# sandyz1000/face-landmark-detector

Measured on AMD Instinct MI355X. Metric: faces/sec (whole node), 256x256 batch inference: fused preprocess + FCN-8 forward + softmax + top-4 landmark decode + similarity/alignment warp, higher is better.
Workload: dtype f32; 1 GPU; BASELINE configs[1]: batch=64/GPU 256x256x3 uint8 crops, fcn_8(68) vanilla encoder fp32, random-init weights (seed 2), decode top-4 thresh 0, align to 256x256; global_batch=64, parallelism=dp1

## Files before the change

### face-landmark-detector_amd/csrc/flm_api.hip

```cpp
#include <cmath>
#include <cstdarg>
#include <cstdio>
#include <cstring>

#include "flm_common.h"

namespace flm {

static thread_local char g_err[512] = "";

void set_error(const char* fmt, ...) {
  va_list ap;
  va_start(ap, fmt);
  vsnprintf(g_err, sizeof(g_err), fmt, ap);
  va_end(ap);
}

int hip_fail(hipError_t e, const char* what) {
  set_error("HIP error %d (%s) at %s", (int)e, hipGetErrorString(e), what);
  return FLM_ERR_HIP;
}

struct Knob {
  const char* key;
// ... 6 lines not shown
    {"bf16_lds_dma", {1}, nullptr, nullptr},
    {"bf16_mfma16", {1}, nullptr, nullptr},
    {"bf16_halo_mfma16", {1}, nullptr, nullptr},
    {"f32_two_level", {1}, nullptr, nullptr},
    {"f32_lean_tile", {1}, nullptr, nullptr},
    {"bf16_group_n", {0}, [](int v) { return v >= 0 && v <= 32 && !(v & (v - 1)); }, "0 or a power of two <= 32"},
    {"bf16_conv3_halo", {1}, nullptr, nullptr},
    {"bf16_score1x1", {1}, nullptr, nullptr},
    {"bf16_fused_tail", {1}, nullptr, nullptr},
    {"decode_lds_dma", {1}, nullptr, nullptr},
    {"posmajor_order", {1}, nullptr, nullptr},
    {"warp_rows", {1}, [](int v) { return v == 0 || v == 1 || v == 4; }, "0, 1 or 4"},
    {"up3_cand8", {1}, [](int v) { return v >= 0 && v <= 7; }, "in [0,7]"},
    {"up3_cand8_rows", {0}, [](int v) { return v >= 0 && v <= 8 && !(v & (v - 1)); }, "0, 1, 2, 4 or 8"},
    {"up3_wreg", {0}, [](int v) { return v == 0 || v == 1; }, "0 or 1"},
};
static_assert(sizeof(g_knobs) / sizeof(g_knobs[0]) == KNOB_COUNT, "one row per KnobId");
int tuning(KnobId id) { return g_knobs[id].value.load(std::memory_order_relaxed); }
static Knob* find_knob(const char* who, const char* key) {
  for (Knob& k : g_knobs)
    if (!strcmp(k.key, key)) return &k;
  set_error("%s: unknown key '%s'", who, key);
  return nullptr;
}

struct ProfRec {
  const char* name;
  hipEvent_t a, b;
};
static ProfRec* g_prof = nullptr;
// ... 182 lines not shown
    t.ho = 2 * hi; t.wo = 2 * wi; t.ldy = L.g.Cp;
  }
  return t;
}

}

using namespace flm;

extern "C" {

int flm_abi_version(void) { return FLM_ABI_VERSION; }

int flm_debug_query(const char* key, int arg) {
  if (key && !strcmp(key, "igemm_occupancy")) return igemm_occupancy((size_t)arg);
  return -1;
}

int flm_set_tuning(const char* key, int value) {
  if (!key) return FLM_ERR_ARG;
  if (!strcmp(key, "none")) return FLM_OK;
  if (!strcmp(key, "landmark_candidates") || !strcmp(key, "candidate_sub_phases") || !strcmp(key, "candidate_cap_div")) {
    set_error("flm_set_tuning: '%s' changes the workspace layout and is a per-call option now: pass flm_forward_opts to "
              "flm_fcn_workspace_bytes_opts / flm_fcn_forward_opts", key);
    return FLM_ERR_ARG;
  }
  Knob* k = find_knob("flm_set_tuning", key);
  if (!k) return FLM_ERR_ARG;
  if (k->valid && !k->valid(value)) {
    set_error("flm_set_tuning: %s must be %s", key, k->domain);
// ... 1475 lines not shown
```

### face-landmark-detector_amd/csrc/flm_common.h

```cpp
#pragma once

#include <hip/hip_runtime.h>
#include <stddef.h>
#include <stdint.h>

#include <atomic>
#include <mutex>

#include "flm.h"

namespace flm {

void set_error(const char* fmt, ...);
int hip_fail(hipError_t e, const char* what);

#define FLM_HIP(call)                                            \
  do {                                                           \
    hipError_t e_ = (call);                                      \
    if (e_ != hipSuccess) return ::flm::hip_fail(e_, #call);     \
  } while (0)

#define FLM_LAUNCH_CHECK(what)                                   \
  do {                                                           \
    hipError_t e_ = hipGetLastError();                           \
// ... 93 lines not shown
  size_t splitk_bytes;
  size_t probs;
  size_t decode;
  size_t sub, tau, cand, cand_cnt;
  int cand_cap;
  int cand_sub;
  size_t total;
  int oh, ow;
};
Fcn8Ws fcn8_ws_layout(int n, int h, int w, int C, int dtype, int out_mode, int decode_mode, int n_points,
                      int arch = 0, const flm_forward_opts* opts = nullptr);

enum KnobId {
  KNOB_BF16_BIG_TILES, KNOB_BF16_LDS_DMA, KNOB_BF16_MFMA16, KNOB_BF16_HALO_MFMA16, KNOB_F32_TWO_LEVEL, KNOB_F32_LEAN_TILE,
  KNOB_BF16_GROUP_N, KNOB_BF16_CONV3_HALO, KNOB_BF16_SCORE1X1, KNOB_BF16_FUSED_TAIL, KNOB_DECODE_LDS_DMA,
  KNOB_POSMAJOR_ORDER, KNOB_WARP_ROWS, KNOB_UP3_CAND8, KNOB_UP3_CAND8_ROWS, KNOB_UP3_WREG, KNOB_COUNT
};
int tuning(KnobId id);

int launch_pack_fcn(hipStream_t s, const flm_fcn_params& p, int C, const Fcn8Pack& L, char* blob);

int launch_enc1(hipStream_t s, const void* x, int in_format, int n, int h, int w, const float* w1p,
                const float* scale, const float* shift, void* f1, int out_bf16, int pool);

struct IgemmDesc {
  const void* x;
  const void* wt;
  const float* scale;
  const float* shift;
  void* y;
  int bf16;
  int out_f32;
  int n, h, w, cin;
  int cout;
  int coutpad;
  int ldc;
  int kh, kw, pad;
  int relu, pool, posmajor;
  int stride;
  const void* res;
  float* splitk_ws;
  size_t splitk_ws_bytes;
};
int launch_igemm(hipStream_t s, const IgemmDesc& d);
int igemm_occupancy(size_t lds_bytes);
int launch_seg_fused_bf16(hipStream_t s, const float* fuse4, const void* w4_packed, const void* f3, const void* w3,
                          const float* scale3, const float* shift3, float* seg, int n, int h4, int w4d, int C, int Cp,
                          int G, int cin3, int coutpad3);

struct ConvTDesc {
  const float* x;
  const void* wf;
  const float* skip;
  void* y;
  int n, hi, wi;
  int ho, wo;
  int s;
  int ldy;
  int epilogue;
  ConvTGeom g;
// ... 163 lines not shown
```

### face-landmark-detector_amd/csrc/flm_igemm.hip

```cpp
#include <type_traits>
#include <vector>

#include "flm_igemm_args.h"

#ifndef FLM_IGEMM_VAR
#define FLM_IGEMM_VAR 0
#endif

namespace flm {

typedef float f32x16 __attribute__((ext_vector_type(16)));
typedef __bf16 bf16x8 __attribute__((ext_vector_type(8)));

constexpr int BM = 128, BN = 128, BK = 32;
constexpr int TILE_F = BM * BK;

__device__ __forceinline__ int swz(int row, int chunk) { return row * BK + ((chunk ^ ((row >> 1) & 7)) << 2); }

__device__ __forceinline__ float f4c(const float4& v, int i) { return i == 0 ? v.x : (i == 1 ? v.y : (i == 2 ? v.z : v.w)); }

template <bool BF, int IDX>
__device__ __forceinline__ void mfma_slot(const float4& a0, const float4& a1, const float4& b0, const float4& b1,
                                          f32x16& c00, f32x16& c01, f32x16& c10, f32x16& c11) {
  if constexpr (BF) {
    const float4& av = (IDX >> 1) ? a1 : a0;
    const float4& bv = (IDX & 1) ? b1 : b0;
    const bf16x8 af = __builtin_bit_cast(bf16x8, av), bfr = __builtin_bit_cast(bf16x8, bv);
    if constexpr (IDX == 0) c00 = __builtin_amdgcn_mfma_f32_32x32x16_bf16(af, bfr, c00, 0, 0, 0);
    if constexpr (IDX == 1) c01 = __builtin_amdgcn_mfma_f32_32x32x16_bf16(af, bfr, c01, 0, 0, 0);
    if constexpr (IDX == 2) c10 = __builtin_amdgcn_mfma_f32_32x32x16_bf16(af, bfr, c10, 0, 0, 0);
    if constexpr (IDX == 3) c11 = __builtin_amdgcn_mfma_f32_32x32x16_bf16(af, bfr, c11, 0, 0, 0);
  } else {
    c00 = __builtin_amdgcn_mfma_f32_32x32x2f32(f4c(a0, IDX), f4c(b0, IDX), c00, 0, 0, 0);
    c01 = __builtin_amdgcn_mfma_f32_32x32x2f32(f4c(a0, IDX), f4c(b1, IDX), c01, 0, 0, 0);
    c10 = __builtin_amdgcn_mfma_f32_32x32x2f32(f4c(a1, IDX), f4c(b0, IDX), c10, 0, 0, 0);
    c11 = __builtin_amdgcn_mfma_f32_32x32x2f32(f4c(a1, IDX), f4c(b1, IDX), c11, 0, 0, 0);
  }
}

template <bool BF, int MMAP, bool RELU, bool TWO = false, bool LEAN = false>
__global__ __launch_bounds__(256, 2) void igemm_kernel(IgemmArgs a) {
  static_assert(!TWO || !BF, "the multi-level accumulation is the fp32 (parity) form");
  static_assert(!LEAN || (TWO && MMAP != 2), "the lean set-up / write-out is built for the fp32 form, row-major and quad order");
  constexpr int ES = BF ? 2 : 4;
  constexpr int EPC = 16 / ES;
  extern __shared__ __attribute__((aligned(16))) char smem_raw[];
  float* As = reinterpret_cast<float*>(smem_raw);
  float* Bs = As + 2 * TILE_F;
  unsigned long long* s_mask = reinterpret_cast<unsigned long long*>(Bs + 2 * TILE_F);

  const int tid = threadIdx.x;
  const int lane = tid & 63;
  const int wave = tid >> 6;
  const int L = xcd_remap(blockIdx.x, gridDim.x);
  constexpr bool PAIR = (MMAP == 2) && !TWO;
  const int mslots = PAIR ? (a.mtiles + 1) / 2 : a.mtiles;
  int mslot = L % mslots, nt = L / mslots;
  if (MMAP == 2 && TWO && (a.ntiles & 7) == 0) {
    const int ppx = a.ntiles >> 3, per_xcd = mslots * ppx;
    const int xcd = L / per_xcd, l = L - xcd * per_xcd;
    mslot = l / ppx;
    nt = xcd * ppx + (l - mslot * ppx);
  }
  const int n0 = nt * BN;
  const int npass = (PAIR && mslot != a.mtiles - 1 - mslot) ? 2 : 1;
  int pair_mt[2] = {mslot, mslot};
  if (MMAP == 2) {
    unsigned long long* tmask = reinterpret_cast<unsigned long long*>(As);
    int* wk = reinterpret_cast<int*>(tmask + a.mtiles);
    int* ord = wk + a.mtiles;
    for (int t = tid; t < a.mtiles; t += 256) tmask[t] = 0ull;
    __syncthreads();
    const int npp = (BM - 1) / a.n + 2;
    for (int idx = tid; idx < a.mtiles * npp; idx += 256) {
      const int t = idx / npp, m_lo = t * BM, m_hi = (m_lo + BM < a.M ? m_lo + BM : a.M) - 1;
      const int p = m_lo / a.n + (idx - t * npp);
      if (p <= m_hi / a.n) atomicOr(&tmask[t], posmajor_posmask(posmajor_pos(a, p), a.h, a.w, a.kh, a.kw, a.pad));
    }
    __syncthreads();
    for (int t = tid; t < a.mtiles; t += 256) wk[t] = __builtin_popcountll(tmask[t]);
    __syncthreads();
    for (int t = tid; t < a.mtiles; t += 256) {
      const int wt = wk[t];
      int rank = 0;
      for (int u = 0; u < a.mtiles; ++u) rank += (wk[u] > wt) || (wk[u] == wt && u < t);
      ord[rank] = t;
    }
    __syncthreads();
    pair_mt[0] = TWO ? __builtin_amdgcn_readfirstlane(ord[mslot]) : ord[mslot];
    pair_mt[1] = ord[a.mtiles - 1 - mslot];
    __syncthreads();
  }
  for (int pass = 0; pass < npass; ++pass) {
  const int mt = pair_mt[pass];
  const int m0 = mt * BM;
  if (pass) __syncthreads();

  const int c8 = TWO ? ((tid & 7) ^ ((tid >> 4) & 7)) : (tid & 7), r0 = tid >> 3;
  int pn[4], py[4], px[4];
  bool pv[4];
#pragma unroll
  for (int j = 0; j < 4; ++j) {
    const int m = m0 + r0 + 32 * j;
    pv[j] = m < a.M;
    const int mm = pv[j] ? m : 0;
    if constexpr (LEAN) {
      const int q = MMAP == 1 ? mm >> 2 : mm, d = mm & 3;
      const int q1 = igemm_fastdiv(q, a.dx_magic, a.dx_shift), xq = q - q1 * a.dx;
      const int q2 = igemm_fastdiv(q1, a.dy_magic, a.dy_shift), yq = q1 - q2 * a.dy;
      px[j] = MMAP == 1 ? 2 * xq + (d & 1) : xq * a.stride;
      py[j] = MMAP == 1 ? 2 * yq + (d >> 1) : yq * a.stride;
      pn[j] = q2;
    } else if ((FLM_IGEMM_VAR & 64) && MMAP != 2) {
      const int q = MMAP == 1 ? mm >> 2 : mm, d = mm & 3;
      const int lw = __builtin_ctz(MMAP == 1 ? a.w >> 1 : a.wo), lh2 = __builtin_ctz(MMAP == 1 ? a.h >> 1 : a.ho);
      const int xq = q & ((1 << lw) - 1), yq = (q >> lw) & ((1 << lh2) - 1);
      px[j] = MMAP == 1 ? 2 * xq + (d & 1) : xq * a.stride;
// ... 16 lines not shown
    }
  }

  const int ntaps = a.kh * a.kw;
  unsigned long long tapmask;
  if (ntaps == 1) {
    tapmask = 1ull;
  } else if ((LEAN && a.all_taps) || ((FLM_IGEMM_VAR & 64) && !LEAN && MMAP != 2)) {
    tapmask = ntaps >= 64 ? ~0ull : (1ull << ntaps) - 1ull;
  } else {
    unsigned long long mymask = 0;
    for (int t = 0; t < ntaps; ++t) {
      const int ky = t / a.kw - a.pad, kx = t % a.kw - a.pad;
      bool any = false;
#pragma unroll
      for (int j = 0; j < 4; ++j)
        any |= pv[j] && (unsigned)(py[j] + ky) < (unsigned)a.h && (unsigned)(px[j] + kx) < (unsigned)a.w;
      if (__any(any)) mymask |= 1ull << t;
    }
    if (lane == 0) s_mask[wave] = mymask;
    __syncthreads();
    tapmask = s_mask[0] | s_mask[1] | s_mask[2] | s_mask[3];
    const unsigned tm_lo = (unsigned)__builtin_amdgcn_readfirstlane((int)(unsigned)tapmask);
    const unsigned tm_hi = (unsigned)__builtin_amdgcn_readfirstlane((int)(unsigned)(tapmask >> 32));
    tapmask = ((unsigned long long)tm_hi << 32) | (unsigned long long)tm_lo;
  }
  const int ntv = __builtin_popcountll(tapmask);
  int nit = ntv * a.cpt, chunk0 = 0;
  unsigned long long rem0 = tapmask;
  if (a.ksplit > 1) {
    const int dense = ntaps * a.cpt;
// ... 5 lines not shown
      rem0 = from0 & upto1;
      nit = __builtin_popcountll(rem0);
    } else {
      rem0 = from0;
      nit = __builtin_popcountll(from0) + (c1 - c0 - 1) * ntv + __builtin_popcountll(upto1);
    }
    chunk0 = c0;
    if (rem0 == 0ull) {
      rem0 = tapmask;
      ++chunk0;
    }
  }

  unsigned rowoff[4];
#pragma unroll
  for (int j = 0; j < 4; ++j)
    rowoff[j] = ((unsigned)(((pn[j] * a.h + py[j]) * a.w + px[j]) * a.cin) + EPC * c8) * ES;
  const char* wrow[4];
#pragma unroll
  for (int j = 0; j < 4; ++j)
    wrow[j] = reinterpret_cast<const char*>(a.wt) + ((size_t)(n0 + r0 + 32 * j) * a.K + EPC * c8) * ES;
  const char* xbase = reinterpret_cast<const char*>(a.x);

  int fa0, fa1, fb0, fb1, fc0, fc1, fc2, fc3;
#define FLM_FRAG_OFFSETS()                                                                                              \
  {                                                                                                                     \
    const int wr = wave >> 1, wc = wave & 1;                                                                            \
    const int lr = lane & 31, lh = lane >> 5;                                                                           \
    const int swx = (lr >> 1) & 7;                                                                                      \
    fa0 = (64 * wr + lr) * BK, fa1 = fa0 + 32 * BK;                                                                     \
    fb0 = (64 * wc + lr) * BK, fb1 = fb0 + 32 * BK;                                                                     \
    fc0 = ((0 + lh) ^ swx) << 2, fc1 = ((2 + lh) ^ swx) << 2, fc2 = ((4 + lh) ^ swx) << 2, fc3 = ((6 + lh) ^ swx) << 2; \
  }
  if constexpr (!LEAN) FLM_FRAG_OFFSETS()

  f32x16 acc00, acc01, acc10, acc11;
  if constexpr (!LEAN) {
#pragma unroll
    for (int r = 0; r < 16; ++r) acc00[r] = acc01[r] = acc10[r] = acc11[r] = 0.f;
  }

  if constexpr (TWO) {
    f32x16 sum00, sum01, sum10, sum11;
    f32x16 top00, top01, top10, top11;
    f32x16 zero16;
#define FLM_CLEAR_SETS()                                                                                                       \
  _Pragma("unroll") for (int r = 0; r < 16; ++r)                                                                               \
      sum00[r] = sum01[r] = sum10[r] = sum11[r] = top00[r] = top01[r] = top10[r] = top11[r] = zero16[r] = 0.f;
    if constexpr (!LEAN) FLM_CLEAR_SETS()

    typedef __attribute__((address_space(3))) char lds_char;
    const int wave_s = __builtin_amdgcn_readfirstlane(wave);
    const unsigned dma_a = (unsigned)(size_t)((lds_char*)smem_raw) + wave_s * 8 * 128;
    const unsigned dma_b = dma_a + 2 * TILE_F * 4;
    const int xbias = (a.pad * a.w + a.pad) * a.cin * 4;
    const dma_srd xdma = dma_make_srd(reinterpret_cast<const char*>(a.x) - xbias);
    const dma_srd wdma = dma_make_srd(reinterpret_cast<const char*>(a.wt) + (size_t)n0 * a.K * 4);
    const unsigned wrow0 = ((unsigned)r0 * (unsigned)a.K + 4u * c8) * 4u;
    const int wstep = 32 * a.K * 4;
    int pyx[4];
#pragma unroll
    for (int j = 0; j < 4; ++j) pyx[j] = ((pv[j] ? py[j] : 0x7000) << 16) | px[j];

    unsigned long long rem = rem0;
    int cur_chunk = chunk0 < a.cpt ? chunk0 : 0;
    int cur_tap = __builtin_ctzll(rem);
    int ld_ky = 0, ld_kx = 0, ld_delta = 0, ld_koff = 0, ld_gid = 0;
    int g_prev = 0, g_cur = 0, g_nx1 = 0;

#define FLM_TILE_PARAMS()                                                    \
  {                                                                          \
    const int ty = (cur_tap * a.kw_magic) >> 16;                             \
    ld_ky = ty - a.pad;                                                      \
    ld_kx = cur_tap - ty * a.kw - a.pad;                                     \
    ld_delta = (ld_ky * a.w + ld_kx) * a.cin * 4 + xbias + cur_chunk * 128;  \
    ld_koff = cur_tap * a.cin * 4 + cur_chunk * 128;                         \
    ld_gid = ((cur_chunk * ntaps + cur_tap) * a.grp_magic) >> 16;            \
    rem &= rem - 1;                                                          \
    if (rem == 0) {                                                          \
      rem = tapmask;                                                         \
      if (++cur_chunk == a.cpt) cur_chunk = 0;  \
    }                                                                        \
    cur_tap = __builtin_ctzll(rem);                                          \
  }
#define FLM_DMA_A(J, STG)                                                                                    \
  {                                                                                                          \
    const int iy = (pyx[J] >> 16) + ld_ky, ix = (pyx[J] & 0xffff) + ld_kx;                                   \
    const bool ok_ = (unsigned)iy < (unsigned)a.h && (unsigned)ix < (unsigned)a.w;                          \
    dma_load16(xdma, dma_a + (STG) * (TILE_F * 4) + (J) * 32 * 128, ok_ ? rowoff[J] : kOobOffset, ld_delta); \
  }
#define FLM_DMA_B(J, STG) dma_load16(wdma, dma_b + (STG) * (TILE_F * 4) + (J) * 32 * 128, wrow0, (J) * wstep + ld_koff);
#define FLM_READ_FRAGS(AF0, AF1, BF0, BF1, T, STG)                                                          \
  {                                                                                                         \
    int oa_ = off_a, ob_ = off_b;                                                                           \
    if (FLM_IGEMM_VAR & 2) asm volatile("" : "+v"(oa_), "+v"(ob_));  \
    const int fct_ = (T) == 0 ? fc0 : ((T) == 1 ? fc1 : ((T) == 2 ? fc2 : fc3));                            \
    const char* pa_ = !(FLM_IGEMM_VAR & 2) ? smem_raw + (fa0 + fct_) * 4 + (STG) * (TILE_F * 4)             \
                                           : smem_raw + ((oa_ ^ ((T) << 5)) + (STG) * (TILE_F * 4));        \
    const char* pb_ = !(FLM_IGEMM_VAR & 2) ? smem_raw + (fb0 + fct_) * 4 + (STG) * (TILE_F * 4) + 2 * TILE_F * 4 \
                                           : smem_raw + ((ob_ ^ ((T) << 5)) + (STG) * (TILE_F * 4) + 2 * TILE_F * 4); \
    AF0 = *reinterpret_cast<const float4*>(pa_);                                                            \
    AF1 = *reinterpret_cast<const float4*>(pa_ + 32 * BK * 4);                                              \
    BF0 = *reinterpret_cast<const float4*>(pb_);                                                            \
    BF1 = *reinterpret_cast<const float4*>(pb_ + 32 * BK * 4);                                              \
  }
#define FLM_SLOT_x 0
#define FLM_SLOT_y 1
#define FLM_SLOT_z 2
#define FLM_SLOT_w 3
#define FLM_MFMA4(AF0, AF1, BF0, BF1, E)                                                     \
  mfma_slot<false, FLM_SLOT_##E>(AF0, AF1, BF0, BF1, acc00, acc01, acc10, acc11);            \
  __builtin_amdgcn_sched_barrier(0);
#define FLM_FLUSH1(SUM, ACC, AV, BV)                                                         \
  SUM += ACC;                                                                                \
  ACC = __builtin_amdgcn_mfma_f32_32x32x2f32(AV, BV, zero16, 0, 0, 0);                       \
  __builtin_amdgcn_sched_barrier(0);
#define FLM_MFMA4_FLUSH(AF0, AF1, BF0, BF1)                                                  \
  FLM_FLUSH1(sum00, acc00, AF0.x, BF0.x)                                                     \
  FLM_FLUSH1(sum01, acc01, AF0.x, BF1.x)                                                     \
  FLM_FLUSH1(sum10, acc10, AF1.x, BF0.x)                                                     \
  FLM_FLUSH1(sum11, acc11, AF1.x, BF1.x)

#define FLM_STEP2(BUF)                                                                                \
  {                                                                                                   \
    FLM_TILE_PARAMS()                                                                                 \
    __builtin_amdgcn_sched_barrier(0);                                                                \
                                  \
    FLM_MFMA4_FLUSH(afx0, afx1, bfx0, bfx1)                                                           \
    FLM_READ_FRAGS(afy0, afy1, bfy0, bfy1, 1, BUF)                                                    \
    FLM_MFMA4(afx0, afx1, bfx0, bfx1, y)                                                              \
    FLM_MFMA4(afx0, afx1, bfx0, bfx1, z)                                                              \
    FLM_MFMA4(afx0, afx1, bfx0, bfx1, w)                                                              \
                                                                                         \
    FLM_MFMA4(afy0, afy1, bfy0, bfy1, x) FLM_READ_FRAGS(afx0, afx1, bfx0, bfx1, 2, BUF)               \
    FLM_MFMA4(afy0, afy1, bfy0, bfy1, y)                                                              \
    FLM_MFMA4(afy0, afy1, bfy0, bfy1, z)                                                              \
    FLM_MFMA4(afy0, afy1, bfy0, bfy1, w)                                                              \
     \
                    \
    FLM_MFMA4(afx0, afx1, bfx0, bfx1, x) FLM_READ_FRAGS(afy0, afy1, bfy0, bfy1, 3, BUF)               \
    FLM_MFMA4(afx0, afx1, bfx0, bfx1, y)                                                              \
    FLM_MFMA4(afx0, afx1, bfx0, bfx1, z)                                                              \
    FLM_MFMA4(afx0, afx1, bfx0, bfx1, w)                                                              \
    if (!(FLM_IGEMM_VAR & 4)) __builtin_amdgcn_s_waitcnt(0x0f70);                                     \
    if (!(FLM_IGEMM_VAR & 16)) __syncthreads();                                                       \
     \
                                                             \
    if (!(FLM_IGEMM_VAR & 1) && g_prev != g_cur) {                                                    \
      top00 += sum00; top01 += sum01; top10 += sum10; top11 += sum11;                                 \
      sum00 = zero16; sum01 = zero16; sum10 = zero16; sum11 = zero16;                                 \
    }                                                                                                 \
     \
    {                                                                                                 \
      FLM_MFMA4(afy0, afy1, bfy0, bfy1, x)                                                            \
      FLM_READ_FRAGS(afx0, afx1, bfx0, bfx1, 0, (BUF) ^ 1)                                            \
      if (!(FLM_IGEMM_VAR & 8)) { FLM_DMA_A(0, BUF) FLM_DMA_B(0, BUF) }                               \
      FLM_MFMA4(afy0, afy1, bfy0, bfy1, y) if (!(FLM_IGEMM_VAR & 8)) { FLM_DMA_A(1, BUF) FLM_DMA_B(1, BUF) } \
      FLM_MFMA4(afy0, afy1, bfy0, bfy1, z) if (!(FLM_IGEMM_VAR & 8)) { FLM_DMA_A(2, BUF) FLM_DMA_B(2, BUF) } \
      FLM_MFMA4(afy0, afy1, bfy0, bfy1, w) if (!(FLM_IGEMM_VAR & 8)) { FLM_DMA_A(3, BUF) FLM_DMA_B(3, BUF) } \
    }                                                                                                 \
    g_prev = g_cur;                                                                                   \
    g_cur = g_nx1;                                                                                    \
    g_nx1 = ld_gid;                                                                                   \
  }

// ... 7 lines not shown
      FLM_DMA_A(0, 1) FLM_DMA_A(1, 1) FLM_DMA_A(2, 1) FLM_DMA_A(3, 1)
      FLM_DMA_B(0, 1) FLM_DMA_B(1, 1) FLM_DMA_B(2, 1) FLM_DMA_B(3, 1)
    }
    if constexpr (LEAN) {
      __builtin_amdgcn_sched_barrier(0);
      FLM_FRAG_OFFSETS()
#pragma unroll
      for (int r = 0; r < 16; ++r) acc00[r] = acc01[r] = acc10[r] = acc11[r] = 0.f;
      FLM_CLEAR_SETS()
    }
    const int off_a = (fa0 + fc0) * 4, off_b = (fb0 + fc0) * 4;
    __builtin_amdgcn_s_waitcnt(0x0f70);
    __syncthreads();
    float4 afx0, afx1, bfx0, bfx1, afy0, afy1, bfy0, bfy1;
    afy0 = afy1 = bfy0 = bfy1 = make_float4(0.f, 0.f, 0.f, 0.f);
    FLM_READ_FRAGS(afx0, afx1, bfx0, bfx1, 0, 0)
    for (int it = 0; it < nit; it += 2) {
      FLM_STEP2(0)
      if (it + 1 < nit) FLM_STEP2(1)
    }
    __builtin_amdgcn_s_waitcnt(0x0f70);
    acc00 = top00 + (sum00 + acc00);
    acc01 = top01 + (sum01 + acc01);
    acc10 = top10 + (sum10 + acc10);
    acc11 = top11 + (sum11 + acc11);
#undef FLM_TILE_PARAMS
#undef FLM_DMA_A
#undef FLM_DMA_B
#undef FLM_READ_FRAGS
#undef FLM_MFMA4
#undef FLM_FLUSH1
#undef FLM_MFMA4_FLUSH
#undef FLM_SLOT_x
#undef FLM_SLOT_y
#undef FLM_SLOT_z
#undef FLM_SLOT_w
#undef FLM_STEP2
#undef FLM_CLEAR_SETS
    if (FLM_IGEMM_VAR & 32) {
      asm volatile("" ::"v"(acc00), "v"(acc01), "v"(acc10), "v"(acc11));
// ... 198 lines not shown
                (yt + row_off)[lane_off] = u;
              }
        };
        if (a.res) store_tile(std::true_type());
        else store_tile(std::false_type());
      }
      continue;
    }
  }
#pragma unroll
  for (int j = 0; j < 2; ++j) {
    const int col = n0 + 64 * wc + 32 * j + lr;
    const bool cok = col < a.cout;
    const float sc = a.scale[col], sh = a.shift[col];
#pragma unroll
    for (int i = 0; i < 2; ++i) {
      const int mbase = m0 + 64 * wr + 32 * i;
      if (MMAP == 1 && a.ksplit > 1) {
#pragma unroll
        for (int r = 0; r < 16; ++r) {
          const int m = mbase + (r & 3) + 8 * (r >> 2) + 4 * lh;
          if (cok && m < a.M) a.part[((size_t)blockIdx.y * a.M + m) * a.ldc + col] = acc[i][j][r];
        }
      } else if (MMAP == 1) {
#pragma unroll
        for (int g = 0; g < 4; ++g) {
          float v = -3.402823466e38f;
#pragma unroll
          for (int e = 0; e < 4; ++e) {
            float u = fmaf(acc[i][j][4 * g + e], sc, sh);
            if (RELU) u = fminf(fmaxf(u, 0.f), a.relu_max);
            v = fmaxf(v, u);
// ... 45 lines not shown
}
bool posperm_cache_get(PospermEntry& e) {
  std::lock_guard<std::mutex> lock(g_posperm_mu);
  for (const PospermEntry& c : g_posperm_cache)
    if (posperm_same(c, e)) { e = c; return true; }
  return false;
}
void posperm_cache_put(const PospermEntry& e) {
  std::lock_guard<std::mutex> lock(g_posperm_mu);
  for (const PospermEntry& c : g_posperm_cache)
    if (posperm_same(c, e)) return;
  if (g_posperm_cache.size() < 64) g_posperm_cache.push_back(e);
}


template <bool BF, int MMAP, bool RELU, bool TWO = false, bool LEAN = false>
static int launch_t(hipStream_t s, const IgemmArgs& a_in) {
  IgemmArgs a = a_in;
  if (MMAP == 2) posmajor_fill_perm(a, BM);
  if (LEAN) igemm_fill_lean(a, MMAP == 1, BM);
  const size_t lds = sizeof(float) * 4 * TILE_F + 64;
  static FuncAttrOnce attr;
  FLM_FUNC_ATTR_ONCE(attr, (&igemm_kernel<BF, MMAP, RELU, TWO, LEAN>), lds);
  const int mslots = (MMAP == 2 && !TWO) ? (a.mtiles + 1) / 2 : a.mtiles;
  igemm_kernel<BF, MMAP, RELU, TWO, LEAN><<<dim3(mslots * a.ntiles, a.ksplit > 1 ? a.ksplit : 1), 256, lds, s>>>(a);
  FLM_LAUNCH_CHECK("igemm_kernel");
  return FLM_OK;
}

__global__ void splitk_reduce_kernel(const float* __restrict__ part, const float* __restrict__ scale,
                                     const float* __restrict__ shift, void* __restrict__ y, int M, int ldc, int cout,
                                     int ksplit, int relu, int out_bf16) {
  const size_t total = (size_t)M * ldc;
  for (size_t i = (size_t)blockIdx.x * blockDim.x + threadIdx.x; i < total; i += (size_t)gridDim.x * blockDim.x) {
    const int c = (int)(i % ldc);
    if (c >= cout) continue;
    float v = 0.f;
    for (int s = 0; s < ksplit; ++s) v += part[(size_t)s * total + i];
    v = fmaf(v, scale[c], shift[c]);
    if (relu) v = fmaxf(v, 0.f);
// ... 20 lines not shown
      best = fmaxf(best, v);
    }
    if (out_bf16) reinterpret_cast<unsigned short*>(y)[i] = f2bf(best);
    else reinterpret_cast<float*>(y)[i] = best;
  }
}

int igemm_occupancy(size_t lds_bytes) {
  int nb = -1;
  if (hipOccupancyMaxActiveBlocksPerMultiprocessor(&nb, reinterpret_cast<const void*>(&igemm_kernel<false, 0, true>), 256,
                                                   lds_bytes) != hipSuccess)
    return -1;
  return nb;
}

template <bool BF, bool TWO = false>
static int dispatch(hipStream_t s, const IgemmDesc& d, const IgemmArgs& a) {
  if constexpr (TWO) {
    if (!d.posmajor && tuning(KNOB_F32_LEAN_TILE)) {
      if (d.pool) return d.relu ? launch_t<BF, 1, true, TWO, true>(s, a) : launch_t<BF, 1, false, TWO, true>(s, a);
      return d.relu ? launch_t<BF, 0, true, TWO, true>(s, a) : launch_t<BF, 0, false, TWO, true>(s, a);
    }
  }
  if (d.pool) return d.relu ? launch_t<BF, 1, true, TWO>(s, a) : launch_t<BF, 1, false, TWO>(s, a);
  if (d.posmajor) return d.relu ? launch_t<BF, 2, true, TWO>(s, a) : launch_t<BF, 2, false, TWO>(s, a);
  return d.relu ? launch_t<BF, 0, true, TWO>(s, a) : launch_t<BF, 0, false, TWO>(s, a);
}


int launch_igemm(hipStream_t s, const IgemmDesc& d) {
  const int es = d.bf16 ? 2 : 4;
  const int bke = 128 / es;
// ... 148 lines not shown
```

### face-landmark-detector_amd/csrc/flm_igemm_args.h

```cpp
#pragma once
#include "flm_common.h"

namespace flm {

struct IgemmArgs {
  const void* x;
  const void* wt;
  const float* scale;
  const float* shift;
  void* y;
  int out_f32;
  float relu_max;
  int n, h, w, cin;
  int ho, wo, stride;
  const void* res;
  int cout, ldc;
  int kh, kw, pad;
  int M;
  int K;
  int mtiles, ntiles;
  int cpt;
  int kw_magic;
  int ksplit;
  float* part;
// ... 21 lines not shown
}

inline void igemm_fill_lean(IgemmArgs& a, bool quads, int bm) {
  a.dx = quads ? a.w >> 1 : a.wo;
  a.dy = quads ? a.h >> 1 : a.ho;
  igemm_fastdiv_make(a.dx, a.dx_magic, a.dx_shift);
  igemm_fastdiv_make(a.dy, a.dy_magic, a.dy_shift);
  const bool edge_only = a.pad <= a.stride && a.kh >= 2 * a.pad + 1 && a.kw >= 2 * a.pad + 1;
  if (quads)
    a.all_taps = edge_only && a.stride == 1 && a.pad <= 1 && a.kh - 1 - a.pad <= 1 && a.kw - 1 - a.pad <= 1 &&
                 a.h >= 2 && a.w >= 2 && !(a.h & 1) && !(a.w & 1);
  else
    a.all_taps = edge_only && a.ho >= 2 && a.wo >= 2 && a.M % bm == 0 && bm >= 3 * a.wo - 1;
}

__device__ __forceinline__ int posmajor_pos(const IgemmArgs& a, int place) {
  if (!a.posperm_on) return place;
  unsigned long long w = a.posperm[0];
#pragma unroll
  for (int k = 1; k < 8; ++k) w = (place >> 3) == k ? a.posperm[k] : w;
  return (int)((w >> ((place & 7) * 8)) & 0xffull);
}

__device__ __forceinline__ unsigned long long posmajor_tapmask(int t, int M, int n, int h, int w, int kh, int kw,
                                                               int pad, int bm = 128) {
  const int m_lo = t * bm, m_hi = (m_lo + bm < M ? m_lo + bm : M) - 1;
  unsigned long long mask = 0;
  for (int p = m_lo / n; p <= m_hi / n; ++p) {
    const int y = p / w, x = p % w;
    for (int ky = 0; ky < kh; ++ky) {
      if ((unsigned)(y + ky - pad) >= (unsigned)h) continue;
      for (int kx = 0; kx < kw; ++kx)
        if ((unsigned)(x + kx - pad) < (unsigned)w) mask |= 1ull << (ky * kw + kx);
    }
  }
  return mask;
}

__device__ __forceinline__ unsigned long long posmajor_posmask(int p, int h, int w, int kh, int kw, int pad) {
  const int y = p / w, x = p - y * w;
  const int kx_lo = pad - x > 0 ? pad - x : 0, kx_hi = pad + w - 1 - x < kw - 1 ? pad + w - 1 - x : kw - 1;
  const int ky_lo = pad - y > 0 ? pad - y : 0, ky_hi = pad + h - 1 - y < kh - 1 ? pad + h - 1 - y : kh - 1;
  if (kx_hi < kx_lo) return 0ull;
  const unsigned long long row = ((1ull << (kx_hi - kx_lo + 1)) - 1ull) << kx_lo;
  unsigned long long mask = 0ull;
  for (int ky = ky_lo; ky <= ky_hi; ++ky) mask |= row << (ky * kw);
  return mask;
}

__device__ __forceinline__ size_t posmajor_orow(int m, int m_first, int nn0, int pos0, int n, int hw) {
  if (n >= 32) {
    int nn = nn0 + (m - m_first), pos = pos0;
    if (nn >= n) {
      nn -= n;
// ... 78 lines not shown
        for (int p = 0; p < P; ++p) best[p] = order[p];
      }
    }
    bool identity = true;
    for (int i = 0; i < P; ++i) {
      identity = identity && best[i] == i;
      ent.table[i >> 3] |= (unsigned long long)best[i] << ((i & 7) * 8);
    }
    ent.on = identity ? 0 : 1;
    posperm_cache_put(ent);
  }
  a.posperm_on = ent.on;
  for (int k = 0; k < 8; ++k) a.posperm[k] = ent.table[k];
}

__device__ __forceinline__ unsigned short f2bf(float v) { return __builtin_bit_cast(unsigned short, (__bf16)v); }

__device__ __forceinline__ uint2 quad_transpose_bf16(float r0, float r1, float r2, float r3, int q) {
  typedef float f32x2_t __attribute__((ext_vector_type(2)));
  typedef __bf16 bf16x2_t __attribute__((ext_vector_type(2)));
  const unsigned p01 = __builtin_bit_cast(unsigned, __builtin_convertvector((f32x2_t){r0, r1}, bf16x2_t));
  const unsigned p23 = __builtin_bit_cast(unsigned, __builtin_convertvector((f32x2_t){r2, r3}, bf16x2_t));
  const unsigned o01 = (unsigned)__builtin_amdgcn_mov_dpp((int)p01, 0xB1, 0xf, 0xf, true);
  const unsigned o23 = (unsigned)__builtin_amdgcn_mov_dpp((int)p23, 0xB1, 0xf, 0xf, true);
  const unsigned sel = (q & 1) ? 0x03020706u : 0x05040100u;
  const unsigned t01 = __builtin_amdgcn_perm(o01, p01, sel);
  const unsigned t23 = __builtin_amdgcn_perm(o23, p23, sel);
  const bool low = q < 2;
  const unsigned recv = (unsigned)__builtin_amdgcn_mov_dpp((int)(low ? t23 : t01), 0x4E, 0xf, 0xf, true);
  return make_uint2(low ? t01 : recv, low ? recv : t23);
// ... 23 lines not shown
```

Before: 7773 faces/s.

## Add 64-row M tiles for fp32 position-major igemm chosen by makespan model

Adds a 64-row M-tile variant of the fp32 two-level position-major implicit-GEMM kernel (half the A tile, two MFMA chains per wave instead of four, smaller LDS, higher launch-bound occupancy). A host-side model estimates per-XCD makespan from tap masks and occupancy for 64- vs 128-row tiles and picks the smaller, cached per shape. The aim is better load balance and CU fill on small-spatial layers like fc6, where few 128-row tiles leave CUs idle. The cost is lower per-wave MFMA reuse, some host-side planning on first call, and one more kernel instantiation.

New measurement: 7896 faces/s (median of 6 runs). +1.6%, better.

```diff
diff --git a/face-landmark-detector_amd/csrc/flm_api.hip b/face-landmark-detector_amd/csrc/flm_api.hip
--- a/face-landmark-detector_amd/csrc/flm_api.hip
+++ b/face-landmark-detector_amd/csrc/flm_api.hip
@@ -44,6 +44,7 @@
     {"up3_cand8", {1}, [](int v) { return v >= 0 && v <= 7; }, "in [0,7]"},
     {"up3_cand8_rows", {0}, [](int v) { return v >= 0 && v <= 8 && !(v & (v - 1)); }, "0, 1, 2, 4 or 8"},
     {"up3_wreg", {0}, [](int v) { return v == 0 || v == 1; }, "0 or 1"},
+    {"f32_fc6_rows", {0}, [](int v) { return v == 0 || v == 64 || v == 128; }, "0, 64 or 128"},
 };
 static_assert(sizeof(g_knobs) / sizeof(g_knobs[0]) == KNOB_COUNT, "one row per KnobId");
 int tuning(KnobId id) { return g_knobs[id].value.load(std::memory_order_relaxed); }
@@ -256,6 +257,7 @@
 
 int flm_debug_query(const char* key, int arg) {
   if (key && !strcmp(key, "igemm_occupancy")) return igemm_occupancy((size_t)arg);
+  if (key && !strcmp(key, "igemm_posmajor_rows")) return igemm_posmajor_rows_last();
   return -1;
 }
 
diff --git a/face-landmark-detector_amd/csrc/flm_common.h b/face-landmark-detector_amd/csrc/flm_common.h
--- a/face-landmark-detector_amd/csrc/flm_common.h
+++ b/face-landmark-detector_amd/csrc/flm_common.h
@@ -131,7 +131,8 @@
 enum KnobId {
   KNOB_BF16_BIG_TILES, KNOB_BF16_LDS_DMA, KNOB_BF16_MFMA16, KNOB_BF16_HALO_MFMA16, KNOB_F32_TWO_LEVEL, KNOB_F32_LEAN_TILE,
   KNOB_BF16_GROUP_N, KNOB_BF16_CONV3_HALO, KNOB_BF16_SCORE1X1, KNOB_BF16_FUSED_TAIL, KNOB_DECODE_LDS_DMA,
-  KNOB_POSMAJOR_ORDER, KNOB_WARP_ROWS, KNOB_UP3_CAND8, KNOB_UP3_CAND8_ROWS, KNOB_UP3_WREG, KNOB_COUNT
+  KNOB_POSMAJOR_ORDER, KNOB_WARP_ROWS, KNOB_UP3_CAND8, KNOB_UP3_CAND8_ROWS, KNOB_UP3_WREG, KNOB_F32_FC6_ROWS,
+  KNOB_COUNT
 };
 int tuning(KnobId id);
 
@@ -161,6 +162,7 @@
 };
 int launch_igemm(hipStream_t s, const IgemmDesc& d);
 int igemm_occupancy(size_t lds_bytes);
+int igemm_posmajor_rows_last();
 int launch_seg_fused_bf16(hipStream_t s, const float* fuse4, const void* w4_packed, const void* f3, const void* w3,
                           const float* scale3, const float* shift3, float* seg, int n, int h4, int w4d, int C, int Cp,
                           int G, int cin3, int coutpad3);
diff --git a/face-landmark-detector_amd/csrc/flm_igemm.hip b/face-landmark-detector_amd/csrc/flm_igemm.hip
--- a/face-landmark-detector_amd/csrc/flm_igemm.hip
+++ b/face-landmark-detector_amd/csrc/flm_igemm.hip
@@ -19,7 +19,7 @@
 
 __device__ __forceinline__ float f4c(const float4& v, int i) { return i == 0 ? v.x : (i == 1 ? v.y : (i == 2 ? v.z : v.w)); }
 
-template <bool BF, int IDX>
+template <bool BF, int IDX, bool HALF = false>
 __device__ __forceinline__ void mfma_slot(const float4& a0, const float4& a1, const float4& b0, const float4& b1,
                                           f32x16& c00, f32x16& c01, f32x16& c10, f32x16& c11) {
   if constexpr (BF) {
@@ -33,20 +33,29 @@
   } else {
     c00 = __builtin_amdgcn_mfma_f32_32x32x2f32(f4c(a0, IDX), f4c(b0, IDX), c00, 0, 0, 0);
     c01 = __builtin_amdgcn_mfma_f32_32x32x2f32(f4c(a0, IDX), f4c(b1, IDX), c01, 0, 0, 0);
-    c10 = __builtin_amdgcn_mfma_f32_32x32x2f32(f4c(a1, IDX), f4c(b0, IDX), c10, 0, 0, 0);
-    c11 = __builtin_amdgcn_mfma_f32_32x32x2f32(f4c(a1, IDX), f4c(b1, IDX), c11, 0, 0, 0);
-  }
-}
-
-template <bool BF, int MMAP, bool RELU, bool TWO = false, bool LEAN = false>
-__global__ __launch_bounds__(256, 2) void igemm_kernel(IgemmArgs a) {
+    if constexpr (!HALF) {
+      c10 = __builtin_amdgcn_mfma_f32_32x32x2f32(f4c(a1, IDX), f4c(b0, IDX), c10, 0, 0, 0);
+      c11 = __builtin_amdgcn_mfma_f32_32x32x2f32(f4c(a1, IDX), f4c(b1, IDX), c11, 0, 0, 0);
+    }
+  }
+}
+
+#ifndef FLM_IGEMM_ROWS64_WAVES
+#define FLM_IGEMM_ROWS64_WAVES 3
+#endif
+template <bool BF, int MMAP, bool RELU, bool TWO = false, bool LEAN = false, int BMT = BM>
+__global__ __launch_bounds__(256, BMT == BM ? 2 : FLM_IGEMM_ROWS64_WAVES) void igemm_kernel(IgemmArgs a) {
   static_assert(!TWO || !BF, "the multi-level accumulation is the fp32 (parity) form");
   static_assert(!LEAN || (TWO && MMAP != 2), "the lean set-up / write-out is built for the fp32 form, row-major and quad order");
+  static_assert(BMT == BM || (BMT == 64 && TWO && MMAP == 2), "64-row tiles are built for the fp32 position-major form");
   constexpr int ES = BF ? 2 : 4;
   constexpr int EPC = 16 / ES;
+  constexpr bool HALF = BMT != BM;
+  constexpr int AJ = BMT / 32;
+  constexpr int TILE_A = BMT * BK;
   extern __shared__ __attribute__((aligned(16))) char smem_raw[];
   float* As = reinterpret_cast<float*>(smem_raw);
-  float* Bs = As + 2 * TILE_F;
+  float* Bs = As + 2 * TILE_A;
   unsigned long long* s_mask = reinterpret_cast<unsigned long long*>(Bs + 2 * TILE_F);
 
   const int tid = threadIdx.x;
@@ -71,9 +80,9 @@
     int* ord = wk + a.mtiles;
     for (int t = tid; t < a.mtiles; t += 256) tmask[t] = 0ull;
     __syncthreads();
-    const int npp = (BM - 1) / a.n + 2;
+    const int npp = (BMT - 1) / a.n + 2;
     for (int idx = tid; idx < a.mtiles * npp; idx += 256) {
-      const int t = idx / npp, m_lo = t * BM, m_hi = (m_lo + BM < a.M ? m_lo + BM : a.M) - 1;
+      const int t = idx / npp, m_lo = t * BMT, m_hi = (m_lo + BMT < a.M ? m_lo + BMT : a.M) - 1;
       const int p = m_lo / a.n + (idx - t * npp);
       if (p <= m_hi / a.n) atomicOr(&tmask[t], posmajor_posmask(posmajor_pos(a, p), a.h, a.w, a.kh, a.kw, a.pad));
     }
@@ -93,14 +102,14 @@
   }
   for (int pass = 0; pass < npass; ++pass) {
   const int mt = pair_mt[pass];
-  const int m0 = mt * BM;
+  const int m0 = mt * BMT;
   if (pass) __syncthreads();
 
   const int c8 = TWO ? ((tid & 7) ^ ((tid >> 4) & 7)) : (tid & 7), r0 = tid >> 3;
   int pn[4], py[4], px[4];
   bool pv[4];
 #pragma unroll
-  for (int j = 0; j < 4; ++j) {
+  for (int j = 0; j < AJ; ++j) {
     const int m = m0 + r0 + 32 * j;
     pv[j] = m < a.M;
     const int mm = pv[j] ? m : 0;
@@ -147,7 +156,7 @@
       const int ky = t / a.kw - a.pad, kx = t % a.kw - a.pad;
       bool any = false;
 #pragma unroll
-      for (int j = 0; j < 4; ++j)
+      for (int j = 0; j < AJ; ++j)
         any |= pv[j] && (unsigned)(py[j] + ky) < (unsigned)a.h && (unsigned)(px[j] + kx) < (unsigned)a.w;
       if (__any(any)) mymask |= 1ull << t;
     }
@@ -183,7 +192,7 @@
 
   unsigned rowoff[4];
 #pragma unroll
-  for (int j = 0; j < 4; ++j)
+  for (int j = 0; j < AJ; ++j)
     rowoff[j] = ((unsigned)(((pn[j] * a.h + py[j]) * a.w + px[j]) * a.cin) + EPC * c8) * ES;
   const char* wrow[4];
 #pragma unroll
@@ -197,7 +206,7 @@
     const int wr = wave >> 1, wc = wave & 1;                                                                            \
     const int lr = lane & 31, lh = lane >> 5;                                                                           \
     const int swx = (lr >> 1) & 7;                                                                                      \
-    fa0 = (64 * wr + lr) * BK, fa1 = fa0 + 32 * BK;                                                                     \
+    fa0 = ((BMT / 2) * wr + lr) * BK, fa1 = fa0 + 32 * BK;                                                              \
     fb0 = (64 * wc + lr) * BK, fb1 = fb0 + 32 * BK;                                                                     \
     fc0 = ((0 + lh) ^ swx) << 2, fc1 = ((2 + lh) ^ swx) << 2, fc2 = ((4 + lh) ^ swx) << 2, fc3 = ((6 + lh) ^ swx) << 2; \
   }
@@ -221,7 +230,7 @@
     typedef __attribute__((address_space(3))) char lds_char;
     const int wave_s = __builtin_amdgcn_readfirstlane(wave);
     const unsigned dma_a = (unsigned)(size_t)((lds_char*)smem_raw) + wave_s * 8 * 128;
-    const unsigned dma_b = dma_a + 2 * TILE_F * 4;
+    const unsigned dma_b = dma_a + 2 * TILE_A * 4;
     const int xbias = (a.pad * a.w + a.pad) * a.cin * 4;
     const dma_srd xdma = dma_make_srd(reinterpret_cast<const char*>(a.x) - xbias);
     const dma_srd wdma = dma_make_srd(reinterpret_cast<const char*>(a.wt) + (size_t)n0 * a.K * 4);
@@ -229,7 +238,7 @@
     const int wstep = 32 * a.K * 4;
     int pyx[4];
 #pragma unroll
-    for (int j = 0; j < 4; ++j) pyx[j] = ((pv[j] ? py[j] : 0x7000) << 16) | px[j];
+    for (int j = 0; j < AJ; ++j) pyx[j] = ((pv[j] ? py[j] : 0x7000) << 16) | px[j];
 
     unsigned long long rem = rem0;
     int cur_chunk = chunk0 < a.cpt ? chunk0 : 0;
@@ -253,10 +262,10 @@
     cur_tap = __builtin_ctzll(rem);                                          \
   }
 #define FLM_DMA_A(J, STG)                                                                                    \
-  {                                                                                                          \
+  if constexpr ((J) < AJ) {                                                                                  \
     const int iy = (pyx[J] >> 16) + ld_ky, ix = (pyx[J] & 0xffff) + ld_kx;                                   \
     const bool ok_ = (unsigned)iy < (unsigned)a.h && (unsigned)ix < (unsigned)a.w;                          \
-    dma_load16(xdma, dma_a + (STG) * (TILE_F * 4) + (J) * 32 * 128, ok_ ? rowoff[J] : kOobOffset, ld_delta); \
+    dma_load16(xdma, dma_a + (STG) * (TILE_A * 4) + (J) * 32 * 128, ok_ ? rowoff[J] : kOobOffset, ld_delta); \
   }
 #define FLM_DMA_B(J, STG) dma_load16(wdma, dma_b + (STG) * (TILE_F * 4) + (J) * 32 * 128, wrow0, (J) * wstep + ld_koff);
 #define FLM_READ_FRAGS(AF0, AF1, BF0, BF1, T, STG)                                                          \
@@ -264,12 +273,12 @@
     int oa_ = off_a, ob_ = off_b;                                                                           \
     if (FLM_IGEMM_VAR & 2) asm volatile("" : "+v"(oa_), "+v"(ob_));  \
     const int fct_ = (T) == 0 ? fc0 : ((T) == 1 ? fc1 : ((T) == 2 ? fc2 : fc3));                            \
-    const char* pa_ = !(FLM_IGEMM_VAR & 2) ? smem_raw + (fa0 + fct_) * 4 + (STG) * (TILE_F * 4)             \
-                                           : smem_raw + ((oa_ ^ ((T) << 5)) + (STG) * (TILE_F * 4));        \
-    const char* pb_ = !(FLM_IGEMM_VAR & 2) ? smem_raw + (fb0 + fct_) * 4 + (STG) * (TILE_F * 4) + 2 * TILE_F * 4 \
-                                           : smem_raw + ((ob_ ^ ((T) << 5)) + (STG) * (TILE_F * 4) + 2 * TILE_F * 4); \
+    const char* pa_ = !(FLM_IGEMM_VAR & 2) ? smem_raw + (fa0 + fct_) * 4 + (STG) * (TILE_A * 4)             \
+                                           : smem_raw + ((oa_ ^ ((T) << 5)) + (STG) * (TILE_A * 4));        \
+    const char* pb_ = !(FLM_IGEMM_VAR & 2) ? smem_raw + (fb0 + fct_) * 4 + (STG) * (TILE_F * 4) + 2 * TILE_A * 4 \
+                                           : smem_raw + ((ob_ ^ ((T) << 5)) + (STG) * (TILE_F * 4) + 2 * TILE_A * 4); \
     AF0 = *reinterpret_cast<const float4*>(pa_);                                                            \
-    AF1 = *reinterpret_cast<const float4*>(pa_ + 32 * BK * 4);                                              \
+    if constexpr (!HALF) AF1 = *reinterpret_cast<const float4*>(pa_ + 32 * BK * 4);                         \
     BF0 = *reinterpret_cast<const float4*>(pb_);                                                            \
     BF1 = *reinterpret_cast<const float4*>(pb_ + 32 * BK * 4);                                              \
   }
@@ -278,7 +287,7 @@
 #define FLM_SLOT_z 2
 #define FLM_SLOT_w 3
 #define FLM_MFMA4(AF0, AF1, BF0, BF1, E)                                                     \
-  mfma_slot<false, FLM_SLOT_##E>(AF0, AF1, BF0, BF1, acc00, acc01, acc10, acc11);            \
+  mfma_slot<false, FLM_SLOT_##E, HALF>(AF0, AF1, BF0, BF1, acc00, acc01, acc10, acc11);      \
   __builtin_amdgcn_sched_barrier(0);
 #define FLM_FLUSH1(SUM, ACC, AV, BV)                                                         \
   SUM += ACC;                                                                                \
@@ -287,8 +296,10 @@
 #define FLM_MFMA4_FLUSH(AF0, AF1, BF0, BF1)                                                  \
   FLM_FLUSH1(sum00, acc00, AF0.x, BF0.x)                                                     \
   FLM_FLUSH1(sum01, acc01, AF0.x, BF1.x)                                                     \
-  FLM_FLUSH1(sum10, acc10, AF1.x, BF0.x)                                                     \
-  FLM_FLUSH1(sum11, acc11, AF1.x, BF1.x)
+  if constexpr (!HALF) {                                                                     \
+    FLM_FLUSH1(sum10, acc10, AF1.x, BF0.x)                                                   \
+    FLM_FLUSH1(sum11, acc11, AF1.x, BF1.x)                                                   \
+  }
 
 #define FLM_STEP2(BUF)                                                                                \
   {                                                                                                   \
@@ -316,8 +327,12 @@
      \
                                                              \
     if (!(FLM_IGEMM_VAR & 1) && g_prev != g_cur) {                                                    \
-      top00 += sum00; top01 += sum01; top10 += sum10; top11 += sum11;                                 \
-      sum00 = zero16; sum01 = zero16; sum10 = zero16; sum11 = zero16;                                 \
+      top00 += sum00; top01 += sum01;                                                                 \
+      sum00 = zero16; sum01 = zero16;                                                                 \
+      if constexpr (!HALF) {                                                                          \
+        top10 += sum10; top11 += sum11;                                                               \
+        sum10 = zero16; sum11 = zero16;                                                               \
+      }                                                                                               \
     }                                                                                                 \
      \
     {                                                                                                 \
@@ -355,6 +370,7 @@
     __syncthreads();
     float4 afx0, afx1, bfx0, bfx1, afy0, afy1, bfy0, bfy1;
     afy0 = afy1 = bfy0 = bfy1 = make_float4(0.f, 0.f, 0.f, 0.f);
+    if constexpr (HALF) afx1 = afy0;
     FLM_READ_FRAGS(afx0, afx1, bfx0, bfx1, 0, 0)
     for (int it = 0; it < nit; it += 2) {
       FLM_STEP2(0)
@@ -363,8 +379,10 @@
     __builtin_amdgcn_s_waitcnt(0x0f70);
     acc00 = top00 + (sum00 + acc00);
     acc01 = top01 + (sum01 + acc01);
-    acc10 = top10 + (sum10 + acc10);
-    acc11 = top11 + (sum11 + acc11);
+    if constexpr (!HALF) {
+      acc10 = top10 + (sum10 + acc10);
+      acc11 = top11 + (sum11 + acc11);
+    }
 #undef FLM_TILE_PARAMS
 #undef FLM_DMA_A
 #undef FLM_DMA_B
@@ -593,8 +611,8 @@
     const bool cok = col < a.cout;
     const float sc = a.scale[col], sh = a.shift[col];
 #pragma unroll
-    for (int i = 0; i < 2; ++i) {
-      const int mbase = m0 + 64 * wr + 32 * i;
+    for (int i = 0; i < BMT / 64; ++i) {
+      const int mbase = m0 + (BMT / 2) * wr + 32 * i;
       if (MMAP == 1 && a.ksplit > 1) {
 #pragma unroll
         for (int r = 0; r < 16; ++r) {
@@ -670,16 +688,22 @@
 }
 
 
-template <bool BF, int MMAP, bool RELU, bool TWO = false, bool LEAN = false>
+template <int BMT>
+constexpr size_t igemm_lds_bytes() {
+  return sizeof(float) * (2 * (BMT == BM || FLM_IGEMM_ROWS64_WAVES == 2 ? BM : BMT) * BK + 2 * TILE_F) + 64;
+}
+
+template <bool BF, int MMAP, bool RELU, bool TWO = false, bool LEAN = false, int BMT = BM>
 static int launch_t(hipStream_t s, const IgemmArgs& a_in) {
   IgemmArgs a = a_in;
-  if (MMAP == 2) posmajor_fill_perm(a, BM);
+  if (BMT != BM) a.mtiles = cdiv(a.M, BMT);
+  if (MMAP == 2) posmajor_fill_perm(a, BMT);
   if (LEAN) igemm_fill_lean(a, MMAP == 1, BM);
-  const size_t lds = sizeof(float) * 4 * TILE_F + 64;
+  const size_t lds = igemm_lds_bytes<BMT>();
   static FuncAttrOnce attr;
-  FLM_FUNC_ATTR_ONCE(attr, (&igemm_kernel<BF, MMAP, RELU, TWO, LEAN>), lds);
+  FLM_FUNC_ATTR_ONCE(attr, (&igemm_kernel<BF, MMAP, RELU, TWO, LEAN, BMT>), lds);
   const int mslots = (MMAP == 2 && !TWO) ? (a.mtiles + 1) / 2 : a.mtiles;
-  igemm_kernel<BF, MMAP, RELU, TWO, LEAN><<<dim3(mslots * a.ntiles, a.ksplit > 1 ? a.ksplit : 1), 256, lds, s>>>(a);
+  igemm_kernel<BF, MMAP, RELU, TWO, LEAN, BMT><<<dim3(mslots * a.ntiles, a.ksplit > 1 ? a.ksplit : 1), 256, lds, s>>>(a);
   FLM_LAUNCH_CHECK("igemm_kernel");
   return FLM_OK;
 }
@@ -730,8 +754,46 @@
   return nb;
 }
 
+struct RowsEntry {
+  int h, w, kh, kw, pad, n, ntiles, dev, rows;
+};
+static std::mutex g_rows_mu;
+static std::vector<RowsEntry> g_rows_cache;
+static std::atomic<int> g_rows_last{0};
+int igemm_posmajor_rows_last() { return g_rows_last.load(std::memory_order_relaxed); }
+
+static int posmajor_rows_for(const IgemmArgs& a) {
+  const int knob = tuning(KNOB_F32_FC6_ROWS);
+  if (knob == 128 || cdiv(a.M, 64) > kRows64MaxTiles) return 128;
+  if (knob == 64) return 64;
+  if (a.ksplit > 1 || a.n >= BM) return 128;
+  int dev = 0;
+  if (hipGetDevice(&dev) != hipSuccess) return 128;
+  std::lock_guard<std::mutex> lock(g_rows_mu);
+  for (const RowsEntry& c : g_rows_cache)
+    if (c.h == a.h && c.w == a.w && c.kh == a.kh && c.kw == a.kw && c.pad == a.pad && c.n == a.n && c.ntiles == a.ntiles && c.dev == dev)
+      return c.rows;
+  int cus = 0, occ128 = 0, occ64 = 0;
+  if (hipDeviceGetAttribute(&cus, hipDeviceAttributeMultiprocessorCount, dev) != hipSuccess ||
+      hipOccupancyMaxActiveBlocksPerMultiprocessor(&occ128, reinterpret_cast<const void*>(&igemm_kernel<false, 2, true, true, false, BM>),
+                                                   256, igemm_lds_bytes<BM>()) != hipSuccess ||
+      hipOccupancyMaxActiveBlocksPerMultiprocessor(&occ64, reinterpret_cast<const void*>(&igemm_kernel<false, 2, true, true, false, 64>),
+                                                   256, igemm_lds_bytes<64>()) != hipSuccess)
+    return 128;
+  const int rows = posmajor_pick_rows(a, cus / 8 * occ128, cus / 8 * occ64);
+  if (g_rows_cache.size() < 256) g_rows_cache.push_back({a.h, a.w, a.kh, a.kw, a.pad, a.n, a.ntiles, dev, rows});
+  return rows;
+}
+
 template <bool BF, bool TWO = false>
 static int dispatch(hipStream_t s, const IgemmDesc& d, const IgemmArgs& a) {
+  if constexpr (TWO) {
+    if (d.posmajor) {
+      const int rows = posmajor_rows_for(a);
+      g_rows_last.store(rows, std::memory_order_relaxed);
+      if (rows == 64) return d.relu ? launch_t<BF, 2, true, TWO, false, 64>(s, a) : launch_t<BF, 2, false, TWO, false, 64>(s, a);
+    }
+  }
   if constexpr (TWO) {
     if (!d.posmajor && tuning(KNOB_F32_LEAN_TILE)) {
       if (d.pool) return d.relu ? launch_t<BF, 1, true, TWO, true>(s, a) : launch_t<BF, 1, false, TWO, true>(s, a);
diff --git a/face-landmark-detector_amd/csrc/flm_igemm_args.h b/face-landmark-detector_amd/csrc/flm_igemm_args.h
--- a/face-landmark-detector_amd/csrc/flm_igemm_args.h
+++ b/face-landmark-detector_amd/csrc/flm_igemm_args.h
@@ -1,4 +1,7 @@
 #pragma once
+#include <algorithm>
+#include <vector>
+
 #include "flm_common.h"
 
 namespace flm {
@@ -59,7 +62,7 @@
     a.all_taps = edge_only && a.ho >= 2 && a.wo >= 2 && a.M % bm == 0 && bm >= 3 * a.wo - 1;
 }
 
-__device__ __forceinline__ int posmajor_pos(const IgemmArgs& a, int place) {
+__host__ __device__ __forceinline__ int posmajor_pos(const IgemmArgs& a, int place) {
   if (!a.posperm_on) return place;
   unsigned long long w = a.posperm[0];
 #pragma unroll
@@ -82,7 +85,7 @@
   return mask;
 }
 
-__device__ __forceinline__ unsigned long long posmajor_posmask(int p, int h, int w, int kh, int kw, int pad) {
+__host__ __device__ __forceinline__ unsigned long long posmajor_posmask(int p, int h, int w, int kh, int kw, int pad) {
   const int y = p / w, x = p - y * w;
   const int kx_lo = pad - x > 0 ? pad - x : 0, kx_hi = pad + w - 1 - x < kw - 1 ? pad + w - 1 - x : kw - 1;
   const int ky_lo = pad - y > 0 ? pad - y : 0, ky_hi = pad + h - 1 - y < kh - 1 ? pad + h - 1 - y : kh - 1;
@@ -191,6 +194,39 @@
   for (int k = 0; k < 8; ++k) a.posperm[k] = ent.table[k];
 }
 
+
+inline unsigned long long posmajor_tile_mask(const IgemmArgs& a, int bm, int t) {
+  const int m_lo = t * bm, m_hi = (m_lo + bm < a.M ? m_lo + bm : a.M) - 1;
+  unsigned long long mask = 0ull;
+  for (int p = m_lo / a.n; p <= m_hi / a.n; ++p) mask |= posmajor_posmask(posmajor_pos(a, p), a.h, a.w, a.kh, a.kw, a.pad);
+  return mask;
+}
+
+inline long long posmajor_makespan(IgemmArgs a, int bm, int slots_per_xcd) {
+  a.mtiles = (a.M + bm - 1) / bm;
+  posmajor_fill_perm(a, bm);
+  std::vector<int> wk((size_t)a.mtiles);
+  for (int t = 0; t < a.mtiles; ++t) wk[(size_t)t] = __builtin_popcountll(posmajor_tile_mask(a, bm, t)) * (bm / 64);
+  std::sort(wk.begin(), wk.end(), [](int x, int y) { return x > y; });
+  const bool by_xcd = (a.ntiles & 7) == 0;
+  const int copies = by_xcd ? a.ntiles >> 3 : 1, rounds = by_xcd ? 1 : a.ntiles;
+  std::vector<long long> load((size_t)(by_xcd ? slots_per_xcd : 8 * slots_per_xcd), 0ll);
+  for (int round = 0; round < rounds; ++round)
+    for (int t = 0; t < a.mtiles; ++t)
+      for (int c = 0; c < copies; ++c) *std::min_element(load.begin(), load.end()) += wk[(size_t)t];
+  return *std::max_element(load.begin(), load.end());
+}
+
+constexpr int kRows64SurchargePermille = 0;
+constexpr int kRows64MaxTiles = 2048;
+
+inline int posmajor_pick_rows(const IgemmArgs& a, int slots128_per_xcd, int slots64_per_xcd) {
+  if (a.ksplit > 1 || a.n >= 128 || (a.M + 63) / 64 > kRows64MaxTiles || slots128_per_xcd < 1 || slots64_per_xcd < 1) return 128;
+  const long long m128 = posmajor_makespan(a, 128, slots128_per_xcd) * slots128_per_xcd,
+                  m64 = posmajor_makespan(a, 64, slots64_per_xcd) * slots64_per_xcd;
+  return m64 * (1000 + kRows64SurchargePermille) < m128 * 1000 ? 64 : 128;
+}
+
 __device__ __forceinline__ unsigned short f2bf(float v) { return __builtin_bit_cast(unsigned short, (__bf16)v); }
 
 __device__ __forceinline__ uint2 quad_transpose_bf16(float r0, float r1, float r2, float r3, int q) {
```
